# FZJ-INM1-BDA/celldetection

Hardware: AMD Instinct MI355X
Metric: tiles/sec (3x512x512) CpnResNeXt101UNet (higher is better)
Workload: dtype bf16

## Files before the change

celldetection_amd/csrc/conv_igemm.hip:

```cpp
#include <algorithm>
#include <atomic>
#include <cstdio>
#include <cstdlib>

#include "cpn_error.h"
#include "cpn_kernels.h"
#include "lds_dma.h"

#ifndef CPN_FP8
#define CPN_FP8 0
#endif
#if CPN_FP8
#define CPN_NS cpn_fp8
#else
#define CPN_NS cpn
#endif

namespace CPN_NS {
using namespace cpn;


#if CPN_FP8
typedef unsigned char elem_t;
#else
// ... 217 lines not shown
    else
        asm volatile(CPN_WAIT_ALL_ASM : "+v"(w[0]), "+v"(p[0]) :: "memory");
}
template <int WN, int WM, int FRAG_STRIDE>
__device__ __forceinline__ void load_frags(frag_t (&w)[WN], frag_t (&p)[WM], unsigned paddr, unsigned waddr) {
    ds_read16<0>(w[0], waddr);
    if constexpr (WN > 1) ds_read16<32 * REC>(w[1], waddr);
    ds_read16<0>(p[0], paddr);
    if constexpr (WM > 1) ds_read16<FRAG_STRIDE>(p[1], paddr);
    if constexpr (WM > 2) {
        ds_read16<2 * FRAG_STRIDE>(p[2], paddr);
        ds_read16<3 * FRAG_STRIDE>(p[3], paddr);
    }
}

template <int WM, int FRAG_STRIDE>
__device__ __forceinline__ void load_pfrags(frag_t (&p)[WM], unsigned paddr) {
    static_assert(WM == 4 || WM == 2, "register-weight loop: 128- or 64-pixel wave tile");
    ds_read16<0>(p[0], paddr);
    ds_read16<FRAG_STRIDE>(p[1], paddr);
    if constexpr (WM > 2) {
        ds_read16<2 * FRAG_STRIDE>(p[2], paddr);
        ds_read16<3 * FRAG_STRIDE>(p[3], paddr);
    }
}
template <int N, int WM>
__device__ __forceinline__ void wait_pfrags(frag_t (&p)[WM]) {
    if constexpr (WM == 4) asm volatile("s_waitcnt lgkmcnt(%4)" : "+v"(p[0]), "+v"(p[1]), "+v"(p[2]), "+v"(p[3]) : "n"(N));
    else asm volatile("s_waitcnt lgkmcnt(%2)" : "+v"(p[0]), "+v"(p[1]) : "n"(N));
}

__host__ __device__ inline int frame_kw(const ConvArgs &a) { return (a.stride == 1 && !a.narrow && a.KW > 1) ? a.KW : 0; }

struct ItemState {
    int c, ky, kx;
};
__device__ __forceinline__ ItemState next_item(const ItemState I, int KH, int KW) {
    ItemState N = I;
    N.kx = I.kx + 1;
    if (N.kx == KW) {
        N.kx = 0;
        N.ky = I.ky + 1;
        if (N.ky == KH) {
            N.ky = 0;
            N.c = I.c + 1;
        }
    }
    return N;
}

#if defined(CPN_EXP_CLOCK) && CPN_EXP_CLOCK == 2 && !CPN_FP8
__device__ unsigned long long g_clock_probe[15];
#endif

template <int TH, int BN, int WM, int WN, int MODE>
__global__ __launch_bounds__((64 * (TH / WM) * (BN / (32 * WN))), ((MODE == MODE_S1F || MODE == MODE_BRF) ? 2 : 1)) void conv_igemm_kernel(const ConvArgs a) {
#if defined(CPN_EXP_CLOCK) && CPN_EXP_CLOCK == 1
    const unsigned long long clk_entry = __builtin_readcyclecounter();
#endif
    using C = Cfg<TH, BN, WM, WN>;
    constexpr int S = ModeCfg<MODE>::S;
    constexpr int PITCH = ModeCfg<MODE>::PITCH;
    constexpr bool PW = MODE == MODE_PW || MODE == MODE_PWR;
    constexpr bool BL = MODE == MODE_BL;
    constexpr bool RW = MODE == MODE_S1R || MODE == MODE_PWR;
    constexpr bool FL = MODE == MODE_S1F || MODE == MODE_BRF || MODE == MODE_S1Q;
    constexpr int IPS = MODE == MODE_S1Q ? 4 : 2;
    constexpr bool BR = MODE == MODE_BR || MODE == MODE_BRF;
    constexpr bool NR = MODE == MODE_N;
    constexpr int RPF = NR ? 2 : 1;
    extern __shared__ __attribute__((aligned(16))) unsigned char smem[];

    const int tid = threadIdx.x;
    const int lane = tid & 63;
    const int wave = __builtin_amdgcn_readfirstlane(tid >> 6);
    const int wave_m = wave / C::WAVES_N;
    const int wave_n = wave % C::WAVES_N;
    constexpr bool prio_wave = C::NWAVES == 8;

    const int tiles_x = (a.Wout + TW - 1) / TW;
    const int tiles_y = (a.Hout + TH - 1) / TH;
    int bid = blockIdx.x;
    int tx, ty, n;
    int yblk = blockIdx.y;
    bool wrap = false;
// ... 90 lines not shown
    static_assert((IPS * C::W_INSTR_ITEM) % C::NWAVES == 0, "weight DMA must divide evenly over the waves");
    int w_k[W_IW];
    int w_m0[W_IW];
    unsigned w_voff[W_IW];
#pragma unroll
    for (int it = 0; it < W_IW; ++it) {
        const int q = wave + it * C::NWAVES;
        const int k = q / C::W_INSTR_ITEM, qi = q % C::W_INSTR_ITEM;
        w_k[it] = k;
        w_m0[it] = ldsW_off + k * WITEM + (qi << 10);
        w_voff[it] = (n0 + qi * 16 + (lane >> 2) < cout_b) ? (unsigned) (qi << 10) + w_dma_lane
                                                           : (w_dma_lane & 63u);
    }
    const unsigned item_bytes = (unsigned) cout_b * REC;
    const rsrc_t rsw = make_rsrc(a.weights, (unsigned) ((size_t) a.bundles * nitems_packed * cout_b * REC));
    unsigned wsoff = (unsigned) (((size_t) g * nitems_packed * cout_b + n0) * REC);

    constexpr int A_INSTR_WAVE = PW ? (TH * 2 + C::NWAVES - 1) / C::NWAVES : 1;
    const bool pw_fast = PW && a.src1 == nullptr && !a.up0;
    unsigned a_voff[A_INSTR_WAVE];
    bool a_ok[A_INSTR_WAVE];
#pragma unroll
    for (int it = 0; it < A_INSTR_WAVE; ++it) {
        int o0 = -1, o1 = -1;
        if (PW) halo_src_offsets<PITCH>(G, wave + it * C::NWAVES, lane, o0, o1);
        a_ok[it] = (wave + it * C::NWAVES) < hinstr;
        a_voff[it] = o0 < 0 ? OOB_LANE : (unsigned) o0 * (unsigned) ES;
    }

    constexpr int FQ = FL ? (((TH - 1 + (MODE == MODE_S1Q ? 7 : 5)) * PITCH * 4 + 63) / 64 + C::NWAVES - 1) / C::NWAVES : 1;
    unsigned f_voff[FQ];
// ... 74 lines not shown
            }                                                                                                  \
        }                                                                                                      \
    }

#define PW_HALO_DMA(CHUNK)                                                                                     \
    {                                                                                                          \
        const int c_ = (CHUNK);                                                                                \
        const unsigned soff_ = (unsigned) (cin0 + c_ * CH) * (unsigned) ES;                                    \
        unsigned char *dstb_ = smem + (c_ & nhb_mask) * halo_buf;                                              \
        _Pragma("unroll") for (int it = 0; it < A_INSTR_WAVE; ++it)                                            \
            if (a_ok[it]) bdma16<CPN_HALO_AUX>(rs0, a_voff[it], soff_, dstb_ + ((wave + it * C::NWAVES) << 10)); \
    }

#define W_DMA(BUF)                                                                                             \
    if constexpr (!RW) {                                                                                       \
        _Pragma("unroll") for (int it = 0; it < W_IW; ++it)                                                    \
            bdma16<CPN_W_AUX>(rsw, w_voff[it], wsoff + (unsigned) w_k[it] * item_bytes, smem + w_m0[it] + (BUF) * WBUF); \
        wsoff += IPS * item_bytes;                                                                             \
    }

    f32x16 acc[WN][WM];
#pragma unroll
    for (int j = 0; j < WN; ++j)
#pragma unroll
        for (int f = 0; f < WM; ++f)
#pragma unroll
            for (int r = 0; r < 16; ++r) acc[j][f][r] = 0.f;

    const int l31 = lane & 31, lhi = lane >> 5;
    constexpr int PSEL = CPN_FP8 ? 2 : 1;
    const unsigned w_lane = (unsigned) ((wave_n * WN * 32 + l31) * REC + (((PSEL * lhi) ^ ((l31 >> 2) & 3)) << 4));
    const int x_lane = (NR ? (l31 & 15) : l31) * S + (wrap ? (l31 >> 4) * (KW - 1) : 0);
    const int row_wave = wave_m * WM * RPF * S;
// ... 12 lines not shown
#define CPN_EXP_H(x)
#else
#define CPN_EXP_H(x) x
#endif
#ifdef CPN_EXP_NOMFMA
#define CPN_EXP_MMA(ACC, A, B) asm volatile("" ::"v"(A), "v"(B))
#else
#define CPN_EXP_MMA(ACC, A, B) ACC = __builtin_amdgcn_mfma_f32_32x32x16_bf16(A, B, ACC, 0, 0, 0)
#endif

#define ITEM_PADDR(C_, KY_, KX_)                                                                               \
    ((unsigned) ((min((C_), nchunks - 1) & nhb_mask) * halo_buf + (row_wave + (KY_)) * (PITCH * REC)) +        \
     (unsigned) ((x_lane + (KX_)) * REC) + (unsigned) (((PSEL * lhi) ^ (((x_lane + (KX_)) >> 2) & 3)) << 4) + nr_lane)
    const unsigned lds0 = (unsigned) (size_t) (__attribute__((address_space(3))) unsigned char *) smem;
#define LOAD_GROUP(WF, PF, PADDR, WADDR) load_frags<WN, WM, FRAG_STRIDE>(WF, PF, lds0 + (PADDR), lds0 + (WADDR))
#define MMA_GROUP(WF, PF, PENDING)                                                                             \
    {                                                                                                          \
        wait_frags<PENDING, WN, WM>(WF, PF);                                                                   \
        _Pragma("unroll") for (int j = 0; j < WN; ++j)                                                         \
            _Pragma("unroll") for (int f = 0; f < WM; ++f) CPN_EXP_MMA(acc[j][f], WF[j], PF[f]);               \
    }
#if CPN_FP8
#define CPN_RARE(X) (X)
#else
#define CPN_RARE(X) __builtin_expect((X), 0)
#endif
#define ISSUE_AT_TRANSITION(IA, ST1, CHUNK_CHANGED)                                                            \
    {                                                                                                          \
        const int idx2_ = IPS * (ST1) + IPS;                                     \
        if (idx2_ < nitems) {                                                                                  \
// ... 79 lines not shown
        unsigned base[NF1];
#pragma unroll
        for (int f = 0; f < NF1; ++f) {
            const int o = f * 32 + l31b;
            ri[f] = o < NPX1 ? o / 17 : 0;
            rj[f] = o < NPX1 ? o - ri[f] * 17 : 0;
            base[f] = (unsigned) ((ri[f] + 1) * PC + rj[f] + 1);
        }
        const int nit1 = 4 * pch;
        const unsigned lds_pin = (unsigned) (size_t) (__attribute__((address_space(3))) unsigned char *) pin;
        const unsigned char *const w1 = (const unsigned char *) a.pre_w + ((size_t) ph * nit1 * 64 + jb0 * 32 + l31b) * REC + (lhib << 4);
        frag_t pa0[NF1], pa1[NF1];
#pragma unroll
        for (int s1 = 0; s1 < 8; ++s1) {
            if (s1 < nit1) {
                frag_t wA[NJ][2];
#pragma unroll
                for (int j = 0; j < NJ; ++j) {
                    const unsigned char *wp = w1 + ((size_t) s1 * 64 + j * 32) * REC;
                    wA[j][0] = *(const frag_t *) wp;
                    wA[j][1] = *(const frag_t *) (wp + 32);
                }
#ifndef CPN_BR_NOSTAGE1
                const int toff = ((s1 >> 1) & 1) * PC + (s1 & 1);
#pragma unroll
                for (int f = 0; f < NF1; ++f) {
                    const unsigned rec = base[f] + toff;
                    const unsigned ad = lds_pin + (unsigned) ((s1 >> 2) * PBUF) + rec * REC + (((unsigned) lhib ^ ((rec >> 2) & 3u)) << 4);
                    ds_read16<0>(pa0[f], ad);
                    ds_read16<0>(pa1[f], ad ^ 32u);
                }
                if constexpr (NF1 == 5)
                    asm volatile("s_waitcnt lgkmcnt(0)" : "+v"(pa0[0]), "+v"(pa0[1]), "+v"(pa0[2]), "+v"(pa0[3]), "+v"(pa0[4]),
                                 "+v"(pa1[0]), "+v"(pa1[1]), "+v"(pa1[2]), "+v"(pa1[3]), "+v"(pa1[4]));
                else
                    asm volatile("s_waitcnt lgkmcnt(0)" : "+v"(pa0[0]), "+v"(pa0[1]), "+v"(pa0[2]), "+v"(pa1[0]), "+v"(pa1[1]), "+v"(pa1[2]));
#pragma unroll
                for (int j = 0; j < NJ; ++j) {
#pragma unroll
// ... 161 lines not shown
#undef CAT8
#else
    if constexpr (RW) {
        frag_t W0a[WN], W0b[WN], W1a[WN], W1b[WN], pA[WM], pB[WM];
        const unsigned wl0 = (unsigned) ((wave_n * WN * 32 + l31) * REC + (lhi << 4)), wl1 = wl0 + 32u;
#define VLOADW(DST, WL, SOFF)                                                                                  \
    _Pragma("unroll") for (int j = 0; j < WN; ++j)                                                             \
        DST[j] = __builtin_bit_cast(frag_t, __builtin_amdgcn_raw_buffer_load_b128(rsw, (int) ((WL) + j * 32 * REC), (int) (SOFF), 0))
#define LOADP(PF, PADDR) load_pfrags<WM, FRAG_STRIDE>(PF, lds0 + (PADDR))
#define MMAP(WF, PF, PENDING)                                                                                  \
    {                                                                                                          \
        wait_pfrags<PENDING, WM>(PF);                                                                          \
        _Pragma("unroll") for (int j = 0; j < WN; ++j)                                                         \
            _Pragma("unroll") for (int f = 0; f < WM; ++f) CPN_EXP_MMA(acc[j][f], WF[j], PF[f]);               \
    }
        unsigned so = wsoff;
        VLOADW(W0a, wl0, so); VLOADW(W0b, wl1, so);
        VLOADW(W1a, wl0, so + item_bytes); VLOADW(W1b, wl1, so + item_bytes);
        unsigned pa = ITEM_PADDR(i0.c, i0.ky, i0.kx);
        LOADP(pA, pa);
        bool land_due = nchunks > 1;
        for (int st = 0; st + 1 < nsteps; ++st) {
            so += 2 * item_bytes;
            LOADP(pB, pa ^ 32u);
            MMAP(W0a, pA, WM);
            VLOADW(W0a, wl0, so);
            pa = ITEM_PADDR(i1.c, i1.ky, i1.kx);
            LOADP(pA, pa);
            MMAP(W0b, pB, WM);
            VLOADW(W0b, wl1, so);
            LOADP(pB, pa ^ 32u);
            MMAP(W1a, pA, WM);
            VLOADW(W1a, wl0, so + item_bytes);
            const ItemState n0i = next_item(i1, KH, KW);
            const bool changed = n0i.c != i0.c;
            if (changed || land_due) {
                wait_pfrags<0, WM>(pB);
                asm volatile("s_waitcnt vmcnt(8)" ::: "memory");
                __builtin_amdgcn_s_barrier();
                land_due = false;
                if constexpr (PW) {
                    const int idx2_ = 2 * (st + 1) + 2;
                    if (idx2_ < nreal) {
                        if (pw_fast) { PW_HALO_DMA(idx2_); } else { HALO_DMA(idx2_); }
                        land_due = true;
                    }
                    if (idx2_ + 1 < nreal) {
                        if (pw_fast) { PW_HALO_DMA(idx2_ + 1); } else { HALO_DMA(idx2_ + 1); }
                    }
                } else if (changed && n0i.c + 1 < nchunks) {
                    HALO_DMA(n0i.c + 1);
                    land_due = true;
                }
            }
            pa = ITEM_PADDR(n0i.c, n0i.ky, n0i.kx);
            LOADP(pA, pa);
            MMAP(W1b, pB, WM);
            VLOADW(W1b, wl1, so + item_bytes);
            wait_pfrags<0, WM>(pA);
            i0 = n0i;
            i1 = next_item(n0i, KH, KW);
        }
        LOADP(pB, pa ^ 32u);
        MMAP(W0a, pA, WM);
        pa = ITEM_PADDR(i1.c, i1.ky, i1.kx);
        LOADP(pA, pa);
        MMAP(W0b, pB, WM);
        LOADP(pB, pa ^ 32u);
        MMAP(W1a, pA, WM);
        MMAP(W1b, pB, 0);
#undef VLOADW
#undef LOADP
#undef MMAP
    } else {
    frag_t wA[WN], pA[WM], wB[WN], pB[WM];
    constexpr int NF = WN + WM;
    unsigned pa = ITEM_PADDR(i0.c, i0.ky, i0.kx);
    unsigned wa = (unsigned) ldsW_off + w_lane;
    LOAD_GROUP(wA, pA, pa, wa);

    if constexpr (IPS == 4) {
    ItemState cur = i0;
#define QSTEP_NEXT() { cur = next_item(cur, KH, KW); pa = ITEM_PADDR(cur.c, cur.ky, cur.kx); wa += WITEM; }
#define QSTEP_HEAD()                                                                                           \
        LOAD_GROUP(wB, pB, pa ^ 32u, wa ^ 32u);                                           \
        MMA_GROUP(wA, pA, NF);                                                             \
        QSTEP_NEXT();                                                                                           \
        LOAD_GROUP(wA, pA, pa, wa);                                                        \
        MMA_GROUP(wB, pB, NF);                                                             \
        LOAD_GROUP(wB, pB, pa ^ 32u, wa ^ 32u);                                           \
        MMA_GROUP(wA, pA, NF);                                                             \
        QSTEP_NEXT();                                                                                           \
        LOAD_GROUP(wA, pA, pa, wa);                                                        \
        MMA_GROUP(wB, pB, NF);                                                             \
        LOAD_GROUP(wB, pB, pa ^ 32u, wa ^ 32u);                                           \
        MMA_GROUP(wA, pA, NF);                                                             \
        QSTEP_NEXT();                                                                                           \
        LOAD_GROUP(wA, pA, pa, wa);                                                        \
        MMA_GROUP(wB, pB, NF);                                                             \
        LOAD_GROUP(wB, pB, pa ^ 32u, wa ^ 32u);                                           \
        MMA_GROUP(wA, pA, NF);
    int c_first = 0;
    for (int st = 0; st + 1 < nsteps; ++st) {
        QSTEP_HEAD();
        cur = next_item(cur, KH, KW);
        wait_all<WN, WM>(wB, pB);
        __builtin_amdgcn_s_barrier();
        ISSUE_AT_TRANSITION(cur, st + 1, cur.c != c_first);
        c_first = cur.c;
        pa = ITEM_PADDR(cur.c, cur.ky, cur.kx);
        wa = (unsigned) (ldsW_off + ((st + 1) & 1) * WBUF) + w_lane;
        LOAD_GROUP(wA, pA, pa, wa);
        MMA_GROUP(wB, pB, NF);
#if CPN_BACKEDGE_WAIT == 1
        wait_frags<0, WN, WM>(wA, pA);
#endif
    }
    QSTEP_HEAD();
    MMA_GROUP(wB, pB, 0);
#undef QSTEP_NEXT
#undef QSTEP_HEAD
    } else {
#define PIN_ACC_ALL()                                                                                          \
    _Pragma("unroll") for (int j_ = 0; j_ < WN; ++j_)                                                          \
        _Pragma("unroll") for (int f_ = 0; f_ < WM; ++f_) asm volatile("" : "+v"(acc[j_][f_]))
    for (int st = 0; st + 1 < nsteps; ++st) {
        LOAD_GROUP(wB, pB, pa ^ 32u, wa ^ 32u);
        MMA_GROUP(wA, pA, NF);
        pa = ITEM_PADDR(i1.c, i1.ky, i1.kx);
        wa += WITEM;
        LOAD_GROUP(wA, pA, pa, wa);
        MMA_GROUP(wB, pB, NF);
        LOAD_GROUP(wB, pB, pa ^ 32u, wa ^ 32u);
        MMA_GROUP(wA, pA, NF);
        const ItemState n0i = next_item(i1, KH, KW);
        wait_all<WN, WM>(wB, pB);
        __builtin_amdgcn_s_barrier();
        ISSUE_AT_TRANSITION(n0i, st + 1, n0i.c != i0.c);
        pa = ITEM_PADDR(n0i.c, n0i.ky, n0i.kx);
        wa = (unsigned) (ldsW_off + ((st + 1) & 1) * WBUF) + w_lane;
        LOAD_GROUP(wA, pA, pa, wa);
        MMA_GROUP(wB, pB, NF);
#if CPN_BACKEDGE_WAIT == 1
        wait_frags<0, WN, WM>(wA, pA);
#elif CPN_BACKEDGE_WAIT == 2
        PIN_ACC_ALL();
        wait_frags<0, WN, WM>(wA, pA);
#endif
        CPN_BL_FLUSH();
        i0 = n0i;
        i1 = next_item(n0i, KH, KW);
    }
    LOAD_GROUP(wB, pB, pa ^ 32u, wa ^ 32u);
    MMA_GROUP(wA, pA, NF);
    pa = ITEM_PADDR(i1.c, i1.ky, i1.kx);
    wa += WITEM;
    LOAD_GROUP(wA, pA, pa, wa);
    MMA_GROUP(wB, pB, NF);
    LOAD_GROUP(wB, pB, pa ^ 32u, wa ^ 32u);
    MMA_GROUP(wA, pA, NF);
    MMA_GROUP(wB, pB, 0);
    }
    }
#endif
#undef HALO_DMA
#undef HALO_DMA_RANGE
#undef HALO_DMA_RANGE_ROWS
#undef CPN_HALO_AT_TRANSITION
#undef CPN_BL_FLUSH
#undef PW_HALO_DMA
#undef W_DMA
#undef LOAD_GROUP
#undef MMA_GROUP
#undef ISSUE_AT_TRANSITION
#undef ITEM_PADDR

#if defined(CPN_EXP_CLOCK) && CPN_EXP_CLOCK == 1
    unsigned long long clk_epi[3] = {0, 0, 0};
#define CPN_EPI_STAMP(I) clk_epi[I] = __builtin_readcyclecounter()
#else
#define CPN_EPI_STAMP(I)
#endif
#ifdef CPN_EXP_CLOCK
    const unsigned long long clk_loop_end = __builtin_readcyclecounter();
    unsigned long long clk_print = 0;
    if (tid == 0 && blockIdx.x == gridDim.x / 2 && blockIdx.y == gridDim.y / 2 && blockIdx.z == 0) {
        const unsigned long long dc = clk_loop_end - clk_c0, dr = __builtin_amdgcn_s_memrealtime() - clk_r0;
// ... 355 lines not shown
    const char *e = getenv("CPN_S1F");
    const int mode = e ? atoi(e) : CPN_S1F_DEFAULT;
    if (mode == 0) return false;
    const bool shape = a.stride == 1 && a.KH >= 2 && a.KH <= 5 && a.KW >= 2 && a.KW <= 5 && !a.src1 && !a.up0 && !a.up1 &&
                       a.region == 0 && !a.narrow && a.out_mode == OUT_BF16_NHWC && a.cout_b % 128 == 0 && a.Hout >= 8;
    if (!shape) return false;
    const size_t halo_buf = (size_t) (((8 - 1 + a.KH) * 36 * 4 + 63) / 64) * 1024;
    if ((a.cin_b / 32 > 1 ? 2 : 1) * halo_buf + 2 * 2 * (size_t) 128 * REC > 160 * 1024 / 2) return false;
    const long blocks = (long) ((a.Wout + TW - 1) / TW) * ((a.Hout + 7) / 8) * a.N * (a.cout_b / 128) * a.bundles;
    return mode == 2 || blocks >= 1024;
}

static bool quad_ok(const ConvArgs &a) {
    if (CPN_FP8) return false;
    const char *e = getenv("CPN_S1Q");
    if (e && atoi(e) == 0) return false;
    return a.stride == 1 && a.KH == a.KW && (a.KH == 5 || a.KH == 7) && !a.src1 && !a.up0 && !a.up1 && a.region == 0 && !a.narrow &&
           a.phase == 0 && a.bundles == 1 && a.cout_b == 64 && a.Hout >= 16 &&
           (a.out_mode == OUT_BF16_NHWC || a.out_mode == OUT_FUSED_HEAD) &&
           (long) ((a.Wout + TW - 1) / TW) * ((a.Hout + 15) / 16) * a.N >= 448;
}

static int conv_mode(const ConvArgs &a) {
    if (a.pre_src) return MODE_BR;
    if (quad_ok(a)) return MODE_S1Q;
    if (a.narrow) return MODE_N;
    if (flat_ok(a)) return MODE_S1F;
    if (a.KH == 1 && a.KW == 1 && a.pad == 0) {
        const char *e = getenv("CPN_PWR");
        return (!CPN_FP8 && e && atoi(e) != 0) ? MODE_PWR : MODE_PW;
    }
    if (a.up0 == 2) return MODE_BL;
    if (a.stride == 2) return MODE_S2;
    const char *e = getenv("CPN_RW");
    const int rw = e ? atoi(e) : CPN_RW_DEFAULT;
// ... 91 lines not shown
    constexpr long MIN_BLOCKS = 224;
    if (TH == 8 && blocks(8, BN) < MIN_BLOCKS) TH = 4;
    if (blocks(TH, BN) < MIN_BLOCKS && BN > 128) BN = 128;
    if (blocks(TH, BN) < MIN_BLOCKS && BN > 64) BN = 64;
    while (lds_bytes(a, TH, BN) > LDS_MAX && BN > 32) BN >>= 1;
    const char *e64 = getenv("CPN_TH64");
    if (BN == 64 && TH == 8 && a.Hout >= 16 && lds_bytes(a, 16, 64) <= LDS_MAX && blocks(16, 64) >= 2 * MIN_BLOCKS &&
        !(e64 && atoi(e64) == 8))
        TH = 16;
    if (const char *ep = getenv("CPN_PW_TILE"); ep && a.KH == 1 && a.KW == 1 && a.pad == 0 && a.out_mode == OUT_BF16_NHWC) {
        int th = 0, bn = 0;
        if (sscanf(ep, "%d,%d", &th, &bn) == 2 && (th == 4 || th == 8) && (bn == 64 || bn == 128 || bn == 256) && bn <= a.cout_b &&
            a.Hout >= th && lds_bytes(a, th, bn) <= LDS_MAX)
            return TileChoice{th, bn};
    }
    return TileChoice{TH, BN};
}

static int fused_head_rows(const ConvArgs &a, const TileChoice &c) { return (a.cout_b == 64 && c.TH == 16) ? 16 : 8; }

int launch_conv(const ConvArgs &a_in, hipStream_t stream) {
    ConvArgs a = a_in;
    if (narrow_ok(a)) {
        a.narrow = 1;
        a.Hout /= 2;
        a.Wout = 32;
    }
    if (a.cin_b % CH || a.cout_b % 32 || a.c0_used % CH) return (int) hipErrorInvalidValue;
    if (a.phase == 3 && (a.out_mode != OUT_FUSED_HEAD || a.bundles != 4 || a.stride != 1)) return (int) hipErrorInvalidValue;
    if ((a.region == 1 || a.region == 2) ? (a.out_mode != OUT_FUSED_HEAD || a.region_margin < 0) : a.region != 0)
        return (int) hipErrorInvalidValue;
    if (a.stride != 1 && a.stride != 2 && !(a.KH == 1 && a.KW == 1 && a.pad == 0 && a.stride >= 1)) return (int) hipErrorInvalidValue;
    if (a.up0 == 2 && (CPN_FP8 || a.stride != 1 || a.src1 || a.up1 || (a.KH == 1 && a.KW == 1)))
        return (int) hipErrorInvalidValue;
    if ((a.stride == 1 && a.KW > 17) || (a.stride == 2 && a.KW > 18)) return (int) hipErrorInvalidValue;
#if !CPN_FP8
    if (a.pre_src) {
// ... 73 lines not shown
```

celldetection_amd/csrc/conv_pair.hip:

```cpp
#include <atomic>
#include <cstdlib>

#include "cpn_kernels.h"
#include "lds_dma.h"

namespace cpn {
namespace {

typedef bf16x8 frag_t;

template <int WLOG, int SL>
struct PairCfg {
    static constexpr bool GEN = WLOG == 0;
    static constexpr int W = GEN ? 34 : (1 << WLOG);
    static constexpr int WC = SL / 64;
    static constexpr int WP = 8 / WC;
    static constexpr int NF1 = 5 * WP;
    static constexpr int NPXP = NF1 * 32;
    static constexpr int ROWS = (GEN || W == 16) ? 18 : NPXP / W;
    static constexpr int NPX = ROWS * W;
    static constexpr int THO = ROWS - 2;
    static constexpr int TWO = GEN ? 32 : W;
    static constexpr int OUTF = THO * TWO / 32;
    static constexpr int PQ = OUTF / 4;
// ... 216 lines not shown
#undef PAIR_MMA
#undef PAIR_DMA

    const int jp = wave / C::PQ, pq = wave % C::PQ;
    constexpr int COB = 32 * CB;
    constexpr int NI2 = 9 * CB + ((9 * CB) & 1);
    const unsigned char *wrow[2];
#pragma unroll
    for (int j = 0; j < 2; ++j) {
        const int bundle = CB == 1 ? (n0 >> 5) + jp * 2 + j : (n0 >> 6) + jp;
        const int row = CB == 1 ? l31 : j * 32 + l31;
        wrow[j] = (const unsigned char *) a.w2 + ((size_t) bundle * NI2 * COB + row) * 64 + lhi * 16;
    }
    frag_t Wr[3][2];
#define PAIR_G_S(G) ((G) / 18)
#define PAIR_G_TAP(G) (((G) % 18) >> 1)
#define PAIR_G_KH(G) ((G) & 1)
#define PAIR_LOADW(G)                                                                                          \
    {                                                                                                          \
        constexpr int s_ = PAIR_G_S(G), t_ = PAIR_G_TAP(G), kh_ = PAIR_G_KH(G);                                \
        if constexpr (CB == 1) {                                                                               \
            Wr[(G) % 3][0] = *(const frag_t *) (wrow[s_] + t_ * (COB * 64) + kh_ * 32);                        \
        } else {                                                                                               \
            Wr[(G) % 3][0] = *(const frag_t *) (wrow[0] + (s_ * 9 + t_) * (COB * 64) + kh_ * 32);              \
            Wr[(G) % 3][1] = *(const frag_t *) (wrow[1] + (s_ * 9 + t_) * (COB * 64) + kh_ * 32);              \
        }                                                                                                      \
    }
#ifndef PAIR_EXP_NOS2
    PAIR_LOADW(0);
    PAIR_LOADW(1);
#endif
// ... 24 lines not shown
            }
        }
    }
    __syncthreads();

    if constexpr (STRIDE == 2) {
        f32x16 a2[2];
#pragma unroll
        for (int j = 0; j < 2; ++j)
#pragma unroll
            for (int r = 0; r < 16; ++r) a2[j][r] = 0.f;
        const unsigned u2 = (unsigned) ((4 * pq + 2 * (l31 >> 4)) * 34 + 2 * (l31 & 15));
        const unsigned base2 = lds0 + (unsigned) (jp * 2 * XB);
        frag_t P2[2];
        auto p2_addr = [&](int g) -> unsigned {
            const int s_ = g / 18, t_ = (g % 18) >> 1, kh_ = g & 1;
            const unsigned tt = u2 + (unsigned) ((t_ / 3) * 34 + t_ % 3);
            return base2 + (unsigned) (s_ * XB) + tt * 64u + ((((unsigned) lhi ^ ((tt >> 2) & 3u)) << 4) ^ (unsigned) (kh_ * 32));
        };
#ifndef PAIR_EXP_NOS2
        ds_read16<0>(P2[0], p2_addr(0));
#pragma unroll
        for (int g = 0; g < 36; ++g) {
            const int s_ = g / 18, t_ = (g % 18) >> 1, kh_ = g & 1;
            if (g + 2 < 36) {
                const int s2_ = (g + 2) / 18, t2_ = ((g + 2) % 18) >> 1, k2_ = (g + 2) & 1;
                if constexpr (CB == 1) {
                    Wr[(g + 2) % 3][0] = *(const frag_t *) (wrow[s2_] + t2_ * (COB * 64) + k2_ * 32);
                } else {
                    Wr[(g + 2) % 3][0] = *(const frag_t *) (wrow[0] + (s2_ * 9 + t2_) * (COB * 64) + k2_ * 32);
                    Wr[(g + 2) % 3][1] = *(const frag_t *) (wrow[1] + (s2_ * 9 + t2_) * (COB * 64) + k2_ * 32);
                }
            }
            if (g + 1 < 36) {
                ds_read16<0>(P2[(g + 1) & 1], p2_addr(g + 1));
                asm volatile("s_waitcnt lgkmcnt(1)" : "+v"(P2[g & 1]));
            } else {
                asm volatile("s_waitcnt lgkmcnt(0)" : "+v"(P2[g & 1]));
            }
            (void) t_; (void) kh_;
            if constexpr (CB == 1) {
// ... 93 lines not shown
            } else {                                                                                           \
                acc2[0][f] = __builtin_amdgcn_mfma_f32_32x32x16_bf16(Wr[(G) % 3][0], pv, acc2[0][f], 0, 0, 0); \
                acc2[1][f] = __builtin_amdgcn_mfma_f32_32x32x16_bf16(Wr[(G) % 3][1], pv, acc2[1][f], 0, 0, 0); \
            }                                                                                                  \
        }                                                                                                      \
    }
#define PAIR_G4(G) PAIR_GROUP(G) PAIR_GROUP((G) + 1) PAIR_GROUP((G) + 2) PAIR_GROUP((G) + 3)
    PAIR_G4(0) PAIR_G4(4) PAIR_G4(8) PAIR_G4(12) PAIR_G4(16) PAIR_G4(20) PAIR_G4(24) PAIR_G4(28) PAIR_G4(32)
#endif
#undef PAIR_G4
#undef PAIR_GROUP
#undef PAIR_LOADW
#undef PAIR_LOADP
#undef PAIR_G_S
#undef PAIR_G_TAP
#undef PAIR_G_KH

    __syncthreads();
    constexpr int SP = 144;
    lds_u8 *const stg = (lds_u8 *) smem + wave * (32 * SP);
    float4 b2[2][4];
#pragma unroll
    for (int j = 0; j < 2; ++j)
#pragma unroll
        for (int q = 0; q < 4; ++q)
            b2[j][q] = a.b2 ? *(const float4 *) (a.b2 + n0 + jp * 64 + j * 32 + 8 * q + 4 * lhi) : make_float4(0.f, 0.f, 0.f, 0.f);
    const int px_l = lane >> 3, part_l = lane & 7;
    const long img_px = (long) a.H * Wimg;
    unsigned char *const dst_n = (unsigned char *) a.dst + ((size_t) n * img_px * a.dst_stride + n0 + jp * 64 + part_l * 8) * 2;
#pragma unroll
// ... 120 lines not shown
```

celldetection_amd/csrc/cpn_kernels.h:

```cpp
#pragma once
#include <hip/hip_runtime.h>
#include <stdint.h>

namespace cpn {

enum OutMode : int { OUT_BF16_NHWC = 0, OUT_F32_NCHW = 1, OUT_FUSED_HEAD = 2 };
enum Act : int { ACT_NONE = 0, ACT_RELU = 1, ACT_SIGMOID = 2, ACT_TANH_SCALED = 3,
                 ACT_LEAKY_RELU = 4, ACT_SILU = 5, ACT_GELU = 6, ACT_ELU = 7, ACT_TANH = 8, ACT_HARDSWISH = 9, ACT_MISH = 10,
                 ACT_SELU = 11, ACT_SOFTPLUS = 12 };
__host__ __device__ inline float act_apply(float x, int act) {
    switch (act) {
        case ACT_RELU: return fmaxf(x, 0.f);
        case ACT_SIGMOID: return 1.f / (1.f + expf(-x));
        case ACT_LEAKY_RELU: return x > 0.f ? x : 0.01f * x;
        case ACT_SILU: return x / (1.f + expf(-x));
        case ACT_GELU: return 0.5f * x * (1.f + erff(x * 0.70710678118654752440f));
        case ACT_ELU: return x > 0.f ? x : expm1f(x);
        case ACT_TANH: return tanhf(x);
        case ACT_HARDSWISH: return x * fminf(fmaxf(x + 3.f, 0.f), 6.f) / 6.f;
        case ACT_MISH: return x * tanhf(x > 20.f ? x : log1pf(expf(x)));
        case ACT_SELU: return 1.0507009873554804934193349852946f * (x > 0.f ? x : 1.6732632423543772848170429916717f * expm1f(x));
        case ACT_SOFTPLUS: return x > 20.f ? x : log1pf(expf(x));
        default: return x;
    }
// ... 4 lines not shown
    int c0_stride, c1_stride;
    int c0_used;
    int up0, up1;
    int Hs0, Ws0, Hs1, Ws1;
    float sy0, sx0, sy1, sx1;
    int N, Hin, Win;
    int Hout, Wout;
    int KH, KW, stride, pad;
    int bundles;
    int cin_b, cout_b;
    const void *weights;
    const float *bias;
    int phase;
    int region, region_margin;
    int narrow;
    const void *res;
    int res_stride, res_up;
    int res_cph;
    int Hr, Wr;
    float ry, rx;
    int act;
    float act_scale;
    int out_mode;
    void *dst;
    int dst_stride, dst_coff;
    int cout_real;
    const void *fuse_w;
    const float *fuse_b;
    int fuse_cout, fuse_act;
    float fuse_scale;
// ... 136 lines not shown
```

celldetection_amd/csrc/sparse_heads.hip:

```cpp
#include <hip/hip_runtime.h>

#include <atomic>

#include "../../include/cpn_hip.h"
#include "cpn_error.h"
#include "cpn_kernels.h"

namespace cpn {
namespace sparse {

typedef __attribute__((ext_vector_type(8))) __bf16 bf16x8;
typedef __attribute__((ext_vector_type(16))) float f32x16;
typedef __attribute__((ext_vector_type(4))) unsigned int u32x4;
typedef __attribute__((ext_vector_type(2))) unsigned int u32x2;
typedef __attribute__((ext_vector_type(2))) __bf16 bf16x2_t;
typedef __attribute__((ext_vector_type(2))) float f32x2_t;
typedef bf16x8 frag_t;

constexpr int REC = 64;
constexpr int MT = 128;
constexpr int WM = MT / 32;
constexpr int NWAVES = 8;
constexpr int SLOT = MT * REC;
constexpr unsigned OOB_LANE = 0x80000000u;
// ... 73 lines not shown
        gx = rem - gy * a.w;
        gcentre = (unsigned) (((b * a.h + gy) * a.w + gx) * a.cs) * 2u + (unsigned) (((lane & 3) ^ ((lane >> 4) & 3)) << 4);
    }
    const rsrc_t rsf = make_rsrc(a.feat, (unsigned) __builtin_amdgcn_readfirstlane(a.N * a.h * a.w * a.cs * 2));
    const rsrc_t rsw = make_rsrc(H.w1, (unsigned) __builtin_amdgcn_readfirstlane((int) (nitems * item_bytes)));
    unsigned char *const gdst = smem + (wave << 10);
#define GATHER(I, C_, KY_, KX_)                                                                                \
    {                                                                                                          \
        const int dy_ = (KY_) - a.pad, dx_ = (KX_) - a.pad;                                                    \
        const bool ok_ = (I) < nreal && (unsigned) (gy + dy_) < (unsigned) a.h && (unsigned) (gx + dx_) < (unsigned) a.w; \
        const unsigned v_ = ok_ ? gcentre + (unsigned) ((dy_ * a.w + dx_) * a.cs * 2) : OOB_LANE;               \
        bdma16(rsf, v_, (unsigned) __builtin_amdgcn_readfirstlane((C_) * 64), gdst + ((I) & 3) * SLOT);         \
    }
    struct It { int c, ky, kx; };
    auto next = [&](It i) {
        if (++i.kx == a.K) { i.kx = 0; if (++i.ky == a.K) { i.ky = 0; ++i.c; } }
        return i;
    };

    f32x16 acc[WN][WM];
#pragma unroll
    for (int j = 0; j < WN; ++j)
#pragma unroll
        for (int f = 0; f < WM; ++f)
#pragma unroll
            for (int r = 0; r < 16; ++r) acc[j][f][r] = 0.f;

    const unsigned wl0 = (unsigned) ((wq * WN * 32 + l31) * REC + (lhi << 4)), wl1 = wl0 + 32u;
    const unsigned lds0 = (unsigned) (size_t) (__attribute__((address_space(3))) unsigned char *) smem;
    const unsigned pl = lds0 + (unsigned) (l31 * REC + ((lhi ^ ((l31 >> 2) & 3)) << 4));
#define VLOADW(DST, WL, SOFF)                                                                                  \
    _Pragma("unroll") for (int j = 0; j < WN; ++j)                                                             \
        DST[j] = __builtin_bit_cast(frag_t, __builtin_amdgcn_raw_buffer_load_b128(rsw, (int) ((WL) + j * 32 * REC), (int) (SOFF), 0))
// ... 4 lines not shown
            _Pragma("unroll") for (int f = 0; f < WM; ++f)                                                     \
                acc[j][f] = __builtin_amdgcn_mfma_f32_32x32x16_bf16(WF[j], PF[f], acc[j][f], 0, 0, 0);         \
    }

    It g0{0, 0, 0};
    It g1 = next(g0);
    GATHER(0, g0.c, g0.ky, g0.kx);
    GATHER(1, g1.c, g1.ky, g1.kx);
    asm volatile("s_waitcnt vmcnt(0)" ::: "memory");
    __builtin_amdgcn_s_barrier();
    g0 = next(g1); g1 = next(g0);
    GATHER(2, g0.c, g0.ky, g0.kx);
    GATHER(3, g1.c, g1.ky, g1.kx);
    asm volatile("" ::: "memory");
    frag_t W0a[WN], W0b[WN], W1a[WN], W1b[WN], pA[WM], pB[WM];
    unsigned so = 0;
    VLOADW(W0a, wl0, so); VLOADW(W0b, wl1, so);
    VLOADW(W1a, wl0, so + item_bytes); VLOADW(W1b, wl1, so + item_bytes);
    load_pfrags(pA, pl);
    for (int st = 0; st + 1 < nsteps; ++st) {
        const unsigned sA = (unsigned) (((2 * st) & 3) * SLOT), sB = (unsigned) (((2 * st + 1) & 3) * SLOT);
        so += 2 * item_bytes;
        load_pfrags(pB, (pl + sA) ^ 32u);
        MMAP(W0a, pA, WM);
        VLOADW(W0a, wl0, so);
        load_pfrags(pA, pl + sB);
        MMAP(W0b, pB, WM);
        VLOADW(W0b, wl1, so);
        load_pfrags(pB, (pl + sB) ^ 32u);
        MMAP(W1a, pA, WM);
        VLOADW(W1a, wl0, so + item_bytes);
        wait_pfrags<0>(pB);
        asm volatile("s_waitcnt vmcnt(%0)" ::"n"(4 * WN) : "memory");
        __builtin_amdgcn_s_barrier();
        if (st + 2 < nsteps) {
            g0 = next(g1); g1 = next(g0);
            GATHER(2 * st + 4, g0.c, g0.ky, g0.kx);
            GATHER(2 * st + 5, g1.c, g1.ky, g1.kx);
        }
        asm volatile("" ::: "memory");
        load_pfrags(pA, pl + (unsigned) (((2 * st + 2) & 3) * SLOT));
        MMAP(W1b, pB, WM);
        VLOADW(W1b, wl1, so + item_bytes);
        wait_pfrags<0>(pA);
    }
    {
        const unsigned sA = (unsigned) (((2 * (nsteps - 1)) & 3) * SLOT), sB = (unsigned) (((2 * (nsteps - 1) + 1) & 3) * SLOT);
        load_pfrags(pB, (pl + sA) ^ 32u);
        MMAP(W0a, pA, WM);
        load_pfrags(pA, pl + sB);
        MMAP(W0b, pB, WM);
        load_pfrags(pB, (pl + sB) ^ 32u);
        MMAP(W1a, pA, WM);
        MMAP(W1b, pB, 0);
    }
#undef GATHER
#undef VLOADW
#undef MMAP
// ... 117 lines not shown
```

Measured before the change: 592.9.

## Reorder conv taps ky-inner and reuse sliding pixel-fragment window across rows

```diff
diff --git a/celldetection_amd/csrc/conv_igemm.hip b/celldetection_amd/csrc/conv_igemm.hip
--- a/celldetection_amd/csrc/conv_igemm.hip
+++ b/celldetection_amd/csrc/conv_igemm.hip
@@ -255,6 +255,24 @@
     }
 }
 
+template <int WN, int WM, int FRAG_STRIDE>
+__device__ __forceinline__ void load_window(frag_t (&w)[WN], frag_t (&p)[WM], unsigned paddr, unsigned waddr, bool col_start) {
+    static_assert(WM == 4 || WM == 2, "window: 128- or 64-pixel wave tile");
+    if (col_start) {
+        ds_read16<0>(p[0], paddr);
+        if constexpr (WM > 2) {
+            ds_read16<FRAG_STRIDE>(p[1], paddr);
+            ds_read16<2 * FRAG_STRIDE>(p[2], paddr);
+        }
+    } else {
+#pragma unroll
+        for (int f = 0; f + 1 < WM; ++f) p[f] = p[f + 1];
+    }
+    ds_read16<0>(w[0], waddr);
+    if constexpr (WN > 1) ds_read16<32 * REC>(w[1], waddr);
+    ds_read16<(WM - 1) * FRAG_STRIDE>(p[WM - 1], paddr);
+}
+
 template <int WM, int FRAG_STRIDE>
 __device__ __forceinline__ void load_pfrags(frag_t (&p)[WM], unsigned paddr) {
     static_assert(WM == 4 || WM == 2, "register-weight loop: 128- or 64-pixel wave tile");
@@ -278,16 +296,19 @@
 };
 __device__ __forceinline__ ItemState next_item(const ItemState I, int KH, int KW) {
     ItemState N = I;
-    N.kx = I.kx + 1;
-    if (N.kx == KW) {
-        N.kx = 0;
-        N.ky = I.ky + 1;
-        if (N.ky == KH) {
-            N.ky = 0;
+    N.ky = I.ky + 1;
+    if (N.ky == KH) {
+        N.ky = 0;
+        N.kx = I.kx + 1;
+        if (N.kx == KW) {
+            N.kx = 0;
             N.c = I.c + 1;
         }
     }
     return N;
+}
+__device__ __forceinline__ int packed_item(const ItemState I, int flat, int nreal, int ntaps, int KW) {
+    return flat < nreal ? I.c * ntaps + I.ky * KW + I.kx : flat;
 }
 
 #if defined(CPN_EXP_CLOCK) && CPN_EXP_CLOCK == 2 && !CPN_FP8
@@ -310,6 +331,7 @@
     constexpr bool BR = MODE == MODE_BR || MODE == MODE_BRF;
     constexpr bool NR = MODE == MODE_N;
     constexpr int RPF = NR ? 2 : 1;
+    constexpr bool WIN = !CPN_FP8 && WM >= 2 && (MODE == MODE_S1 || MODE == MODE_S1F || MODE == MODE_S1Q);
     extern __shared__ __attribute__((aligned(16))) unsigned char smem[];
 
     const int tid = threadIdx.x;
@@ -430,7 +452,9 @@
     }
     const unsigned item_bytes = (unsigned) cout_b * REC;
     const rsrc_t rsw = make_rsrc(a.weights, (unsigned) ((size_t) a.bundles * nitems_packed * cout_b * REC));
-    unsigned wsoff = (unsigned) (((size_t) g * nitems_packed * cout_b + n0) * REC);
+    const unsigned wsoff = (unsigned) (((size_t) g * nitems_packed * cout_b + n0) * REC);
+    ItemState wi{0, 0, 0};
+    int wflat = 0;
 
     constexpr int A_INSTR_WAVE = PW ? (TH * 2 + C::NWAVES - 1) / C::NWAVES : 1;
     const bool pw_fast = PW && a.src1 == nullptr && !a.up0;
@@ -535,9 +559,17 @@
 
 #define W_DMA(BUF)                                                                                             \
     if constexpr (!RW) {                                                                                       \
-        _Pragma("unroll") for (int it = 0; it < W_IW; ++it)                                                    \
-            bdma16<CPN_W_AUX>(rsw, w_voff[it], wsoff + (unsigned) w_k[it] * item_bytes, smem + w_m0[it] + (BUF) * WBUF); \
-        wsoff += IPS * item_bytes;                                                                             \
+        unsigned wso_[IPS];                                                                                    \
+        _Pragma("unroll") for (int k_ = 0; k_ < IPS; ++k_) {                                                   \
+            wso_[k_] = wsoff + (unsigned) (PW ? wflat + k_ : packed_item(wi, wflat + k_, nreal, ntaps, KW)) * item_bytes; \
+            wi = next_item(wi, KH, KW);                                                                        \
+        }                                                                                                      \
+        wflat += IPS;                                                                                          \
+        _Pragma("unroll") for (int it = 0; it < W_IW; ++it) {                                                  \
+            unsigned s_ = wso_[0];                                                                             \
+            _Pragma("unroll") for (int k_ = 1; k_ < IPS; ++k_) s_ = w_k[it] == k_ ? wso_[k_] : s_;            \
+            bdma16<CPN_W_AUX>(rsw, w_voff[it], s_, smem + w_m0[it] + (BUF) * WBUF);                            \
+        }                                                                                                      \
     }
 
     f32x16 acc[WN][WM];
@@ -580,6 +612,12 @@
      (unsigned) ((x_lane + (KX_)) * REC) + (unsigned) (((PSEL * lhi) ^ (((x_lane + (KX_)) >> 2) & 3)) << 4) + nr_lane)
     const unsigned lds0 = (unsigned) (size_t) (__attribute__((address_space(3))) unsigned char *) smem;
 #define LOAD_GROUP(WF, PF, PADDR, WADDR) load_frags<WN, WM, FRAG_STRIDE>(WF, PF, lds0 + (PADDR), lds0 + (WADDR))
+    const bool tapwin = WIN && a.tapwin && KH >= 2;
+#define LOAD_GROUP_KY(WF, PF, PADDR, WADDR, KY)                                                                \
+    {                                                                                                          \
+        if constexpr (WIN) load_window<WN, WM, FRAG_STRIDE>(WF, PF, lds0 + (PADDR), lds0 + (WADDR), !tapwin || (KY) == 0); \
+        else load_frags<WN, WM, FRAG_STRIDE>(WF, PF, lds0 + (PADDR), lds0 + (WADDR));                          \
+    }
 #define MMA_GROUP(WF, PF, PENDING)                                                                             \
     {                                                                                                          \
         wait_frags<PENDING, WN, WM>(WF, PF);                                                                   \
@@ -689,15 +727,16 @@
 #pragma unroll
         for (int s1 = 0; s1 < 8; ++s1) {
             if (s1 < nit1) {
+                const int ps1 = (s1 & 4) + 2 * (s1 & 1) + ((s1 >> 1) & 1);
                 frag_t wA[NJ][2];
 #pragma unroll
                 for (int j = 0; j < NJ; ++j) {
-                    const unsigned char *wp = w1 + ((size_t) s1 * 64 + j * 32) * REC;
+                    const unsigned char *wp = w1 + ((size_t) ps1 * 64 + j * 32) * REC;
                     wA[j][0] = *(const frag_t *) wp;
                     wA[j][1] = *(const frag_t *) (wp + 32);
                 }
 #ifndef CPN_BR_NOSTAGE1
-                const int toff = ((s1 >> 1) & 1) * PC + (s1 & 1);
+                const int toff = (s1 & 1) * PC + ((s1 >> 1) & 1);
 #pragma unroll
                 for (int f = 0; f < NF1; ++f) {
                     const unsigned rec = base[f] + toff;
@@ -889,14 +928,17 @@
         _Pragma("unroll") for (int j = 0; j < WN; ++j)                                                         \
             _Pragma("unroll") for (int f = 0; f < WM; ++f) CPN_EXP_MMA(acc[j][f], WF[j], PF[f]);               \
     }
-        unsigned so = wsoff;
+#define RW_SOFF(I, FLAT) (wsoff + (unsigned) (PW ? (FLAT) : packed_item(I, FLAT, nreal, ntaps, KW)) * item_bytes)
+        unsigned so = RW_SOFF(i0, 0), so1 = RW_SOFF(i1, 1);
         VLOADW(W0a, wl0, so); VLOADW(W0b, wl1, so);
-        VLOADW(W1a, wl0, so + item_bytes); VLOADW(W1b, wl1, so + item_bytes);
+        VLOADW(W1a, wl0, so1); VLOADW(W1b, wl1, so1);
         unsigned pa = ITEM_PADDR(i0.c, i0.ky, i0.kx);
         LOADP(pA, pa);
         bool land_due = nchunks > 1;
         for (int st = 0; st + 1 < nsteps; ++st) {
-            so += 2 * item_bytes;
+            const ItemState n0i = next_item(i1, KH, KW), n1i = next_item(n0i, KH, KW);
+            so = RW_SOFF(n0i, 2 * st + 2);
+            so1 = RW_SOFF(n1i, 2 * st + 3);
             LOADP(pB, pa ^ 32u);
             MMAP(W0a, pA, WM);
             VLOADW(W0a, wl0, so);
@@ -906,8 +948,7 @@
             VLOADW(W0b, wl1, so);
             LOADP(pB, pa ^ 32u);
             MMAP(W1a, pA, WM);
-            VLOADW(W1a, wl0, so + item_bytes);
-            const ItemState n0i = next_item(i1, KH, KW);
+            VLOADW(W1a, wl0, so1);
             const bool changed = n0i.c != i0.c;
             if (changed || land_due) {
                 wait_pfrags<0, WM>(pB);
@@ -931,10 +972,10 @@
             pa = ITEM_PADDR(n0i.c, n0i.ky, n0i.kx);
             LOADP(pA, pa);
             MMAP(W1b, pB, WM);
-            VLOADW(W1b, wl1, so + item_bytes);
+            VLOADW(W1b, wl1, so1);
             wait_pfrags<0, WM>(pA);
             i0 = n0i;
-            i1 = next_item(n0i, KH, KW);
+            i1 = n1i;
         }
         LOADP(pB, pa ^ 32u);
         MMAP(W0a, pA, WM);
@@ -945,35 +986,36 @@
         MMAP(W1a, pA, WM);
         MMAP(W1b, pB, 0);
 #undef VLOADW
+#undef RW_SOFF
 #undef LOADP
 #undef MMAP
     } else {
     frag_t wA[WN], pA[WM], wB[WN], pB[WM];
-    constexpr int NF = WN + WM;
+    constexpr int NF = WIN ? WN + 1 : WN + WM;
     unsigned pa = ITEM_PADDR(i0.c, i0.ky, i0.kx);
     unsigned wa = (unsigned) ldsW_off + w_lane;
-    LOAD_GROUP(wA, pA, pa, wa);
+    LOAD_GROUP_KY(wA, pA, pa, wa, i0.ky);
 
     if constexpr (IPS == 4) {
     ItemState cur = i0;
 #define QSTEP_NEXT() { cur = next_item(cur, KH, KW); pa = ITEM_PADDR(cur.c, cur.ky, cur.kx); wa += WITEM; }
 #define QSTEP_HEAD()                                                                                           \
-        LOAD_GROUP(wB, pB, pa ^ 32u, wa ^ 32u);                                           \
+        LOAD_GROUP_KY(wB, pB, pa ^ 32u, wa ^ 32u, cur.ky);                                      \
         MMA_GROUP(wA, pA, NF);                                                             \
         QSTEP_NEXT();                                                                                           \
-        LOAD_GROUP(wA, pA, pa, wa);                                                        \
+        LOAD_GROUP_KY(wA, pA, pa, wa, cur.ky);                                             \
         MMA_GROUP(wB, pB, NF);                                                             \
-        LOAD_GROUP(wB, pB, pa ^ 32u, wa ^ 32u);                                           \
+        LOAD_GROUP_KY(wB, pB, pa ^ 32u, wa ^ 32u, cur.ky);                                      \
         MMA_GROUP(wA, pA, NF);                                                             \
         QSTEP_NEXT();                                                                                           \
-        LOAD_GROUP(wA, pA, pa, wa);                                                        \
+        LOAD_GROUP_KY(wA, pA, pa, wa, cur.ky);                                             \
         MMA_GROUP(wB, pB, NF);                                                             \
-        LOAD_GROUP(wB, pB, pa ^ 32u, wa ^ 32u);                                           \
+        LOAD_GROUP_KY(wB, pB, pa ^ 32u, wa ^ 32u, cur.ky);                                      \
         MMA_GROUP(wA, pA, NF);                                                             \
         QSTEP_NEXT();                                                                                           \
-        LOAD_GROUP(wA, pA, pa, wa);                                                        \
+        LOAD_GROUP_KY(wA, pA, pa, wa, cur.ky);                                             \
         MMA_GROUP(wB, pB, NF);                                                             \
-        LOAD_GROUP(wB, pB, pa ^ 32u, wa ^ 32u);                                           \
+        LOAD_GROUP_KY(wB, pB, pa ^ 32u, wa ^ 32u, cur.ky);                                      \
         MMA_GROUP(wA, pA, NF);
     int c_first = 0;
     for (int st = 0; st + 1 < nsteps; ++st) {
@@ -985,7 +1027,7 @@
         c_first = cur.c;
         pa = ITEM_PADDR(cur.c, cur.ky, cur.kx);
         wa = (unsigned) (ldsW_off + ((st + 1) & 1) * WBUF) + w_lane;
-        LOAD_GROUP(wA, pA, pa, wa);
+        LOAD_GROUP_KY(wA, pA, pa, wa, cur.ky);
         MMA_GROUP(wB, pB, NF);
 #if CPN_BACKEDGE_WAIT == 1
         wait_frags<0, WN, WM>(wA, pA);
@@ -1000,13 +1042,13 @@
     _Pragma("unroll") for (int j_ = 0; j_ < WN; ++j_)                                                          \
         _Pragma("unroll") for (int f_ = 0; f_ < WM; ++f_) asm volatile("" : "+v"(acc[j_][f_]))
     for (int st = 0; st + 1 < nsteps; ++st) {
-        LOAD_GROUP(wB, pB, pa ^ 32u, wa ^ 32u);
+        LOAD_GROUP_KY(wB, pB, pa ^ 32u, wa ^ 32u, i0.ky);
         MMA_GROUP(wA, pA, NF);
         pa = ITEM_PADDR(i1.c, i1.ky, i1.kx);
         wa += WITEM;
-        LOAD_GROUP(wA, pA, pa, wa);
+        LOAD_GROUP_KY(wA, pA, pa, wa, i1.ky);
         MMA_GROUP(wB, pB, NF);
-        LOAD_GROUP(wB, pB, pa ^ 32u, wa ^ 32u);
+        LOAD_GROUP_KY(wB, pB, pa ^ 32u, wa ^ 32u, i1.ky);
         MMA_GROUP(wA, pA, NF);
         const ItemState n0i = next_item(i1, KH, KW);
         wait_all<WN, WM>(wB, pB);
@@ -1014,7 +1056,7 @@
         ISSUE_AT_TRANSITION(n0i, st + 1, n0i.c != i0.c);
         pa = ITEM_PADDR(n0i.c, n0i.ky, n0i.kx);
         wa = (unsigned) (ldsW_off + ((st + 1) & 1) * WBUF) + w_lane;
-        LOAD_GROUP(wA, pA, pa, wa);
+        LOAD_GROUP_KY(wA, pA, pa, wa, n0i.ky);
         MMA_GROUP(wB, pB, NF);
 #if CPN_BACKEDGE_WAIT == 1
         wait_frags<0, WN, WM>(wA, pA);
@@ -1026,13 +1068,13 @@
         i0 = n0i;
         i1 = next_item(n0i, KH, KW);
     }
-    LOAD_GROUP(wB, pB, pa ^ 32u, wa ^ 32u);
+    LOAD_GROUP_KY(wB, pB, pa ^ 32u, wa ^ 32u, i0.ky);
     MMA_GROUP(wA, pA, NF);
     pa = ITEM_PADDR(i1.c, i1.ky, i1.kx);
     wa += WITEM;
-    LOAD_GROUP(wA, pA, pa, wa);
+    LOAD_GROUP_KY(wA, pA, pa, wa, i1.ky);
     MMA_GROUP(wB, pB, NF);
-    LOAD_GROUP(wB, pB, pa ^ 32u, wa ^ 32u);
+    LOAD_GROUP_KY(wB, pB, pa ^ 32u, wa ^ 32u, i1.ky);
     MMA_GROUP(wA, pA, NF);
     MMA_GROUP(wB, pB, 0);
     }
@@ -1046,6 +1088,7 @@
 #undef PW_HALO_DMA
 #undef W_DMA
 #undef LOAD_GROUP
+#undef LOAD_GROUP_KY
 #undef MMA_GROUP
 #undef ISSUE_AT_TRANSITION
 #undef ITEM_PADDR
@@ -1431,11 +1474,12 @@
 static bool quad_ok(const ConvArgs &a) {
     if (CPN_FP8) return false;
     const char *e = getenv("CPN_S1Q");
-    if (e && atoi(e) == 0) return false;
+    const int mode = e ? atoi(e) : 1;
+    if (mode == 0) return false;
     return a.stride == 1 && a.KH == a.KW && (a.KH == 5 || a.KH == 7) && !a.src1 && !a.up0 && !a.up1 && a.region == 0 && !a.narrow &&
            a.phase == 0 && a.bundles == 1 && a.cout_b == 64 && a.Hout >= 16 &&
            (a.out_mode == OUT_BF16_NHWC || a.out_mode == OUT_FUSED_HEAD) &&
-           (long) ((a.Wout + TW - 1) / TW) * ((a.Hout + 15) / 16) * a.N >= 448;
+           (mode == 2 || (long) ((a.Wout + TW - 1) / TW) * ((a.Hout + 15) / 16) * a.N >= 448);
 }
 
 static int conv_mode(const ConvArgs &a) {
@@ -1557,6 +1601,12 @@
             a.Hout >= th && lds_bytes(a, th, bn) <= LDS_MAX)
             return TileChoice{th, bn};
     }
+    if (const char *ek = getenv("CPN_KK_TILE"); ek && a.KH > 1 && a.KW > 1 && a.out_mode == OUT_BF16_NHWC) {
+        int th = 0, bn = 0;
+        if (sscanf(ek, "%d,%d", &th, &bn) == 2 && (th == 4 || th == 8) && (bn == 64 || bn == 128 || bn == 256) && bn <= a.cout_b &&
+            a.Hout >= th && lds_bytes(a, th, bn) <= LDS_MAX)
+            return TileChoice{th, bn};
+    }
     return TileChoice{TH, BN};
 }
 
@@ -1564,6 +1614,10 @@
 
 int launch_conv(const ConvArgs &a_in, hipStream_t stream) {
     ConvArgs a = a_in;
+    {
+        const char *e = getenv("CPN_TAPWIN");
+        a.tapwin = !(e && atoi(e) == 0);
+    }
     if (narrow_ok(a)) {
         a.narrow = 1;
         a.Hout /= 2;
diff --git a/celldetection_amd/csrc/conv_pair.hip b/celldetection_amd/csrc/conv_pair.hip
--- a/celldetection_amd/csrc/conv_pair.hip
+++ b/celldetection_amd/csrc/conv_pair.hip
@@ -254,7 +254,8 @@
     }
     frag_t Wr[3][2];
 #define PAIR_G_S(G) ((G) / 18)
-#define PAIR_G_TAP(G) (((G) % 18) >> 1)
+#define PAIR_G_POS(G) (((G) % 18) >> 1)
+#define PAIR_G_TAP(G) ((PAIR_G_POS(G) % 3) * 3 + PAIR_G_POS(G) / 3)
 #define PAIR_G_KH(G) ((G) & 1)
 #define PAIR_LOADW(G)                                                                                          \
     {                                                                                                          \
@@ -309,7 +310,7 @@
         const unsigned base2 = lds0 + (unsigned) (jp * 2 * XB);
         frag_t P2[2];
         auto p2_addr = [&](int g) -> unsigned {
-            const int s_ = g / 18, t_ = (g % 18) >> 1, kh_ = g & 1;
+            const int s_ = g / 18, t_ = PAIR_G_TAP(g), kh_ = g & 1;
             const unsigned tt = u2 + (unsigned) ((t_ / 3) * 34 + t_ % 3);
             return base2 + (unsigned) (s_ * XB) + tt * 64u + ((((unsigned) lhi ^ ((tt >> 2) & 3u)) << 4) ^ (unsigned) (kh_ * 32));
         };
@@ -317,9 +318,9 @@
         ds_read16<0>(P2[0], p2_addr(0));
 #pragma unroll
         for (int g = 0; g < 36; ++g) {
-            const int s_ = g / 18, t_ = (g % 18) >> 1, kh_ = g & 1;
+            const int s_ = g / 18, t_ = PAIR_G_TAP(g), kh_ = g & 1;
             if (g + 2 < 36) {
-                const int s2_ = (g + 2) / 18, t2_ = ((g + 2) % 18) >> 1, k2_ = (g + 2) & 1;
+                const int s2_ = (g + 2) / 18, t2_ = PAIR_G_TAP(g + 2), k2_ = (g + 2) & 1;
                 if constexpr (CB == 1) {
                     Wr[(g + 2) % 3][0] = *(const frag_t *) (wrow[s2_] + t2_ * (COB * 64) + k2_ * 32);
                 } else {
@@ -443,6 +444,7 @@
 #undef PAIR_LOADP
 #undef PAIR_G_S
 #undef PAIR_G_TAP
+#undef PAIR_G_POS
 #undef PAIR_G_KH
 
     __syncthreads();
diff --git a/celldetection_amd/csrc/cpn_kernels.h b/celldetection_amd/csrc/cpn_kernels.h
--- a/celldetection_amd/csrc/cpn_kernels.h
+++ b/celldetection_amd/csrc/cpn_kernels.h
@@ -42,6 +42,7 @@
     int phase;
     int region, region_margin;
     int narrow;
+    int tapwin;
     const void *res;
     int res_stride, res_up;
     int res_cph;
diff --git a/celldetection_amd/csrc/sparse_heads.hip b/celldetection_amd/csrc/sparse_heads.hip
--- a/celldetection_amd/csrc/sparse_heads.hip
+++ b/celldetection_amd/csrc/sparse_heads.hip
@@ -111,9 +111,10 @@
     }
     struct It { int c, ky, kx; };
     auto next = [&](It i) {
-        if (++i.kx == a.K) { i.kx = 0; if (++i.ky == a.K) { i.ky = 0; ++i.c; } }
+        if (++i.ky == a.K) { i.ky = 0; if (++i.kx == a.K) { i.kx = 0; ++i.c; } }
         return i;
     };
+    auto slab = [&](It i, int flat) { return (unsigned) (flat < nreal ? (i.c * a.K + i.ky) * a.K + i.kx : flat) * item_bytes; };
 
     f32x16 acc[WN][WM];
 #pragma unroll
@@ -148,13 +149,17 @@
     GATHER(3, g1.c, g1.ky, g1.kx);
     asm volatile("" ::: "memory");
     frag_t W0a[WN], W0b[WN], W1a[WN], W1b[WN], pA[WM], pB[WM];
-    unsigned so = 0;
+    It w0{0, 0, 0};
+    It w1 = next(w0);
+    unsigned so = slab(w0, 0), so1 = slab(w1, 1);
     VLOADW(W0a, wl0, so); VLOADW(W0b, wl1, so);
-    VLOADW(W1a, wl0, so + item_bytes); VLOADW(W1b, wl1, so + item_bytes);
+    VLOADW(W1a, wl0, so1); VLOADW(W1b, wl1, so1);
     load_pfrags(pA, pl);
     for (int st = 0; st + 1 < nsteps; ++st) {
         const unsigned sA = (unsigned) (((2 * st) & 3) * SLOT), sB = (unsigned) (((2 * st + 1) & 3) * SLOT);
-        so += 2 * item_bytes;
+        w0 = next(w1); w1 = next(w0);
+        so = slab(w0, 2 * st + 2);
+        so1 = slab(w1, 2 * st + 3);
         load_pfrags(pB, (pl + sA) ^ 32u);
         MMAP(W0a, pA, WM);
         VLOADW(W0a, wl0, so);
@@ -163,7 +168,7 @@
         VLOADW(W0b, wl1, so);
         load_pfrags(pB, (pl + sB) ^ 32u);
         MMAP(W1a, pA, WM);
-        VLOADW(W1a, wl0, so + item_bytes);
+        VLOADW(W1a, wl0, so1);
         wait_pfrags<0>(pB);
         asm volatile("s_waitcnt vmcnt(%0)" ::"n"(4 * WN) : "memory");
         __builtin_amdgcn_s_barrier();
@@ -175,7 +180,7 @@
         asm volatile("" ::: "memory");
         load_pfrags(pA, pl + (unsigned) (((2 * st + 2) & 3) * SLOT));
         MMAP(W1b, pB, WM);
-        VLOADW(W1b, wl1, so + item_bytes);
+        VLOADW(W1b, wl1, so1);
         wait_pfrags<0>(pA);
     }
     {
```

After: 576.1. 2.8% lower.
